# nubot-nudt/LCR-Net

Measured on AMD Instinct MI355X. Metric: scans/s (120k-pt KITTI-shape scan -> 256-D descriptor), higher is better.
Workload: dtype f32 (K-deep GEMMs, K >= 288 and N >= 64: fp32 operands as bf16 x 3 split, 6 of 9 products on the bf16 matrix cores, fp32 accumulate — error vs fp64 <= the fp32-MFMA kernel's; every other GEMM, KPConv and attention: fp32 MFMA); 1 GPU; configs[1]: batch of 8 synthetic 64-beam scans (~120k pts, 0.3 m voxel -> ~16k pts), voxelise + 3 subsamples + 10 radius searches + KPConv encoder + NetVLAD, seeded random weights; distinct_input_batches=4, streams=pre-processing stream (own host thread, 2 batches ahead) + 2 encoder stream(s), parallelism=scan-parallel x1, all-gather of descriptors

## Files before the change

### include/lcr_hip.h

```cpp
#ifndef LCR_HIP_H
#define LCR_HIP_H
#include <stddef.h>
#include <stdint.h>
#ifdef __cplusplus
extern "C" {
#endif

#define LCR_OK 0
#define LCR_EARG (-1)
#define LCR_ESPACE (-2)
#define LCR_EHIP (-3)

#define LCR_STATUS_KEY_OVERFLOW 1u
#define LCR_STATUS_LEN_MISMATCH 2u
#define LCR_GN_REPLICAS 8

const char* lcr_last_error(void);
void lcr_ktimer_enable(int on);
void lcr_ktimer_sample(int every);
void lcr_ktimer_kinds(unsigned mask);
int lcr_ktimer_read(int kind, int max_records, double* seconds, int64_t* meta);
int lcr_ktimer_read2(int kind, int max_records, double* seconds, double* seconds_kernel, int64_t* meta);
int lcr_stream_spin(int microseconds, void* stream);
int lcr_version(void);
// ... 86 lines not shown
int lcr_gemm_f32_bsplit_masked(const float* A, const uint16_t* Bs_tiles, float* C, int64_t M, int N, int K, const float* bias,
                               const float* rowdiv, const int64_t* seg_len, int S, int groups, double* stats, const uint16_t* row_mask,
                               int block_k, void* stream);
int lcr_kpconv_mask_ok(int64_t M, int N, int K, int split);
int lcr_gemm_f32_anorm(const float* A, const float* B, float* C, int64_t M, int N, int K, const float* bias,
                       const double* a_stats, const float* a_gamma, const float* a_beta, int a_groups, float a_eps,
                       float a_slope, const int64_t* seg_len, int S, int groups, double* stats, void* stream);
int lcr_gemm_f32_bsplit_anorm(const float* A, const uint16_t* Bs_tiles, float* C, int64_t M, int N, int K, const float* bias,
                              const double* a_stats, const float* a_gamma, const float* a_beta, int a_groups, float a_eps,
                              float a_slope, const int64_t* seg_len, int S, int groups, double* stats, void* stream);
int lcr_gemm_split_ok(int N, int K);
int lcr_gemm_f32_batched_ta(const float* A, const float* B, float* C, int64_t M, int N, int count, const int* k_host,
                            const int64_t* a_off_host, const int64_t* b_off_host, const int64_t* c_off_host, void* stream);
int lcr_kpconv_aggregate(const float* s_feats, const uint8_t* s_pos, const float* q_pts, const float* s_pts,
                         const void* idx, int idx_is_64, int64_t M, int64_t Ns, int H, int C,
                         const float* kernel_points_host, float sigma, float* A, float* nn,
                         const int32_t* order , void* stream);
#define LCR_KP_VALID_FIRST 1
int lcr_kpconv_aggregate_ex(const float* s_feats, const uint8_t* s_pos, const float* q_pts, const float* s_pts,
                            const void* idx, int idx_is_64, int64_t M, int64_t Ns, int H, int C,
                            const float* kernel_points_host, float sigma, float* A, float* nn,
                            const int32_t* order, int flags, void* stream);
int lcr_kpconv_aggregate_mask(const float* s_feats, const uint8_t* s_pos, const float* q_pts, const float* s_pts,
                              const void* idx, int idx_is_64, int64_t M, int64_t Ns, int H, int C,
                              const float* kernel_points_host, float sigma, float* A, float* nn, uint16_t* mask,
                              const int32_t* order, int flags, void* stream);
int lcr_kpconv_fused(const float* s_feats, const uint8_t* s_pos, const float* q_pts, const float* s_pts, const void* idx,
                     int idx_is_64, int64_t M, int64_t Ns, int H, int C, const float* kernel_points_host, float sigma,
                     const float* W, const float* bias, float* out, const int64_t* seg_len, int S, int groups, double* stats,
                     const int32_t* order, void* stream);
int lcr_kpconv_cin1(const float* s_feats, const float* q_pts, const float* s_pts, const void* idx, int idx_is_64,
                    int64_t M, int64_t Ns, int H, const float* kernel_points_host, float sigma, const float* W,
                    const float* bias, int Cout, float* out, const int32_t* order, void* stream);
int lcr_maxpool(const float* x, const void* idx, int idx_is_64, int64_t M, int64_t Ns, int H, int C, float* out,
                const int32_t* order, void* stream);
int lcr_row_positive(const float* x, int64_t N, int C, uint8_t* pos, void* stream);
int lcr_groupnorm_stats(const float* x, int64_t N, int C, int groups, const int64_t* seg_len, int S, double* stats, void* stream);
int lcr_groupnorm_apply(const float* x, const double* stats, const float* gamma, const float* beta, const float* res,
                        const double* res_stats, const float* res_gamma, const float* res_beta, float* y, int64_t N, int C,
                        int groups, const int64_t* seg_len, int S, float eps, float slope, int act, uint8_t* pos, void* stream);

#define LCR_ENC_BLOCKS 10
typedef struct LcrUnaryW {
  const float *w, *b;
  const float *gn_w, *gn_b;
  const uint16_t* w_split;
} LcrUnaryW;
typedef struct LcrBlockW {
  int   cin, cout, strided;
  float sigma;
  const float* kernel_points_host;
  const float *kp_w, *kp_b;
  const float* kp_wt;
  const uint16_t* kp_wt_split;
  const float *normconv_w, *normconv_b;
  LcrUnaryW unary1, unary2, shortcut;
} LcrBlockW;
typedef struct LcrEncoderW {
  int   groups, c1_cout;
  float c1_sigma;
  const float* c1_kernel_points_host;
  const float *c1_w, *c1_b;
  const float *c1_gn_w, *c1_gn_b;
  LcrBlockW blocks[LCR_ENC_BLOCKS];
} LcrEncoderW;
int lcr_encoder_ws_bytes(const LcrEncoderW* W, const int64_t* n_host, int S, size_t* bytes);
// ... 222 lines not shown
```

### include/lcr_hip_debug.h

```cpp
#ifndef LCR_HIP_DEBUG_H
#define LCR_HIP_DEBUG_H

#ifdef __cplusplus
extern "C" {
#endif

void lcr_gemm_debug_force_tile(int tile);
void lcr_gemm_debug_deep(int mode);
void lcr_gemm_debug_streamk(int mode);
void lcr_groupnorm_debug_general(int on);
void lcr_kpconv_debug_off64(int on);

#ifdef __cplusplus
}
#endif
#endif
```

### lcr-net_amd/_lib.py

```python
import ctypes
import os
import re
import types

import torch

_PKG = os.path.dirname(os.path.abspath(__file__))
LIB_PATH = os.path.join(_PKG, "liblcr_hip.so")

_lib = None

HEADERS = [os.path.join(_PKG, "..", "include", h) for h in ("lcr_hip.h", "lcr_hip_debug.h")]
_SCALARS = {"int": ctypes.c_int, "int64_t": ctypes.c_int64, "uint32_t": ctypes.c_uint32, "uint64_t": ctypes.c_uint64, "unsigned": ctypes.c_uint,
            "size_t": ctypes.c_size_t, "float": ctypes.c_float, "double": ctypes.c_double}
_RESULTS = {"int": ctypes.c_int, "void": None, "const char*": ctypes.c_char_p}


def parse_header(text):
    text = re.sub(r"/\*.*?\*/|//[^\n]*", " ", text, flags=re.S)
    text = re.sub(r"^\s*#.*$", "", text, flags=re.M)
    sigs = {}
    for m in re.finditer(r"\b(lcr_\w+)\s*\(", text):
        name = m.group(1)
        head = text[:m.start()]
        res = re.sub(r"\s*\*", "*", " ".join(head[max(head.rfind(c) for c in ";{}") + 1:].split()))
        tail = re.match(r"([^()]*)\)\s*;", text[m.end():])
        if res not in _RESULTS or tail is None:
            raise RuntimeError("%s: cannot parse its prototype (result type %r)" % (name, res))
        args = []
        for p in ([] if tail.group(1).strip() in ("", "void") else tail.group(1).split(",")):
            words = re.sub(r"\bconst\b", " ", p).split()
            ctype = ctypes.c_void_p if "*" in p else _SCALARS.get(" ".join(words[:-1] if len(words) > 1 else words))
            if ctype is None:
                raise RuntimeError("%s: parameter %r has no ctypes mapping" % (name, " ".join(p.split())))
            args.append(ctype)
        sigs[name] = (_RESULTS[res], args)
    return sigs


_RELEASES_GIL = {"lcr_roformer_forward", "lcr_precompute_batch", "lcr_precompute_batch_rows", "lcr_precompute_batch_rows_ex", "lcr_hashmap_bucket_host", "lcr_encoder_forward", "lcr_encoder_forward_ex", "lcr_ktimer_read",
                 "lcr_ktimer_read2", "lcr_hashmap_order_host", "lcr_ransac_sample_host", "lcr_icp_point_to_point", "lcr_icp_point_to_plane", "lcr_netvlad_forward", "lcr_log_sinkhorn", "lcr_log_sinkhorn_ex",
                 "lcr_local_global_registration", "lcr_local_global_registration_ex", "lcr_retrieval_topk", "lcr_stream_spin"}


def build():
    import importlib.util
    spec = importlib.util.spec_from_file_location("_lcr_build", os.path.join(_PKG, "csrc", "build.py"))
    mod = importlib.util.module_from_spec(spec)
    spec.loader.exec_module(mod)
    return mod.build()


_RETURNS_VALUE = {"lcr_version", "lcr_kpconv_mask_ok", "lcr_gemm_split_ok", "lcr_ktimer_read", "lcr_ktimer_read2"}


def __getattr__(name):
    if name == "call":
        lib()
        return call
    raise AttributeError(name)


def _raise_on_rc(rc, fn, args):
    if rc:
        check(rc, fn.__name__)
    return rc


def lib():
    global _lib, call
    if _lib is None:
        if not os.path.exists(LIB_PATH):
            raise RuntimeError(
                "liblcr_hip.so not found at %s — build it with `python lcr-net_amd/csrc/build.py` "
                "(there is no CPU fallback for the lcr-net_amd hot path)" % LIB_PATH)
        sigs = {}
        for header in HEADERS:
            with open(header) as f:
                sigs.update(parse_header(f.read()))
        L = ctypes.CDLL(LIB_PATH)
        K = ctypes.PyDLL(LIB_PATH) if os.environ.get("LCR_CTYPES_KEEP_GIL", "1") != "0" else L
        checked = types.SimpleNamespace()
        for name, (res, args) in sigs.items():
            if not hasattr(L, name):
                continue
            dll = L if name in _RELEASES_GIL else K
# ... 46 lines not shown
```

### lcr-net_amd/csrc/encoder.hip

```cpp
#include <algorithm>
#include <cstdlib>
#include <cstring>

#include "common.h"

#define TURN(call) ([&]() { LaunchTurn turn_; return (call); }())

namespace lcr {

constexpr float ENC_GN_EPS = 1e-5f;
constexpr float ENC_SLOPE = 0.1f;

struct Arena {
  char*  base;
  size_t off, cap;
  template <typename T>
  T* take(size_t n) {
    const size_t o = off;
    off = align_up(off + n * sizeof(T));
    return (base && off <= cap) ? reinterpret_cast<T*>(base + o) : nullptr;
  }
};

struct StageIO {
  const float*   pts;
  const int64_t* seg;
  const int32_t* order;
  int64_t        n;
  int64_t        min_rows;
};

struct StatsPool {
  double* base;
  size_t  off, cap;
  int     S, groups;
  double* take() {
    const size_t n = static_cast<size_t>(GN_REPLICAS) * S * groups * 2;
    if (off + n > cap) return nullptr;
    double* p = base + off;
    off += n;
    return p;
  }
};

static size_t stats_doubles(int S, int groups) { return static_cast<size_t>(GN_REPLICAS) * S * groups * 2 * 44; }

static int unary_raw(const LcrUnaryW& u, const float* x, int64_t n, int cin, int cout, const StageIO& st, StatsPool& sp, Arena& ws,
                     float** y_out, double** stats_out, hipStream_t s) {
  float* y = ws.take<float>(static_cast<size_t>(n) * cout);
  double* stats = sp.take();
  if (!y || !stats) return LCR_ESPACE;
  const bool split = u.w_split && lcr_gemm_split_ok(cout, cin);
  int rc = split ? TURN(lcr_gemm_f32_bsplit(x, u.w_split, y, n, cout, cin, u.b, nullptr, st.seg, sp.S, sp.groups, stats, s))
                 : TURN(lcr_gemm_f32(x, u.w, y, n, cout, cin, 0, 1, u.b, nullptr, st.seg, sp.S, sp.groups, stats, s));
  *y_out = y;
  *stats_out = stats;
  return rc;
}

static int residual_block(const LcrBlockW& b, const float* s_feats, const StageIO& q, const StageIO& sup, const void* idx, int H,
                          StatsPool& sp, Arena& ws, float* out, unsigned enc_flags, hipStream_t s) {
  const int mid = b.cout / 4, g = sp.groups;
  const int64_t M = q.n, Ns = sup.n;
  int rc;
  const float* x = s_feats;
  uint8_t* pos = ws.take<uint8_t>(static_cast<size_t>(Ns));
  if (!pos) return LCR_ESPACE;
  if (b.unary1.w) {
    float* y1;
    double* st1;
    if ((rc = unary_raw(b.unary1, s_feats, Ns, b.cin, mid, sup, sp, ws, &y1, &st1, s))) return rc;
    float* x1 = ws.take<float>(static_cast<size_t>(Ns) * mid);
    if (!x1) return LCR_ESPACE;
    if ((rc = TURN(lcr_groupnorm_apply(y1, st1, b.unary1.gn_w, b.unary1.gn_b, nullptr, nullptr, nullptr, nullptr, x1, Ns, mid, g, sup.seg, sp.S,
                                  ENC_GN_EPS, ENC_SLOPE, 1, pos, s))))
      return rc;
    x = x1;
  } else if ((rc = TURN(lcr_row_positive(s_feats, Ns, b.cin, pos, s)))) {
    return rc;
  }
  float* A = ws.take<float>(static_cast<size_t>(M) * 15 * mid);
  float* nn = ws.take<float>(static_cast<size_t>(M));
  float* kpo = ws.take<float>(static_cast<size_t>(M) * mid);
  uint16_t* kmask = ws.take<uint16_t>(static_cast<size_t>(M));
  double* stc = sp.take();
  if (!A || !nn || !kpo || !kmask || !stc) return LCR_ESPACE;
  static const bool vf_env_off = getenv("LCR_KP_VALID_FIRST") && atoi(getenv("LCR_KP_VALID_FIRST")) == 0;
  const int vf_flag = ((enc_flags & LCR_ENC_LISTS_VALID_FIRST) && !vf_env_off) ? LCR_KP_VALID_FIRST : 0;
  static const bool fused32 = getenv("LCR_KPCONV_FUSED") != nullptr;
  if (fused32 && mid == 32 && sp.S <= 64) {
    if ((rc = TURN(lcr_kpconv_fused(x, pos, q.pts, sup.pts, idx, 0, M, Ns, H, mid, b.kernel_points_host, b.sigma, b.kp_w, b.kp_b, kpo, q.seg, sp.S, g,
                                    stc, q.order, s))))
      return rc;
  } else {
    const bool split = b.kp_wt_split && mid >= 64;
    if (!((split || b.kp_wt) && lcr_kpconv_mask_ok(M, mid, 15 * mid, split))) kmask = nullptr;
    if ((rc = TURN(lcr_kpconv_aggregate_mask(x, pos, q.pts, sup.pts, idx, 0, M, Ns, H, mid, b.kernel_points_host, b.sigma, A, nn, kmask, q.order, vf_flag,
                                             s))))
      return rc;
    if (split) {
      if ((rc = TURN(kmask ? lcr_gemm_f32_bsplit_masked(A, b.kp_wt_split, kpo, M, mid, 15 * mid, b.kp_b, nn, q.seg, sp.S, g, stc, kmask, mid, s)
                           : lcr_gemm_f32_bsplit(A, b.kp_wt_split, kpo, M, mid, 15 * mid, b.kp_b, nn, q.seg, sp.S, g, stc, s))))
        return rc;
    } else if (kmask) {
      if ((rc = TURN(lcr_gemm_f32_masked(A, b.kp_wt, kpo, M, mid, 15 * mid, b.kp_b, nn, q.seg, sp.S, g, stc, kmask, mid, s)))) return rc;
    } else if ((rc = TURN(b.kp_wt ? lcr_gemm_f32(A, b.kp_wt, kpo, M, mid, 15 * mid, 0, 1, b.kp_b, nn, q.seg, sp.S, g, stc, s)
                                  : lcr_gemm_f32(A, b.kp_w, kpo, M, mid, 15 * mid, 0, 0, b.kp_b, nn, q.seg, sp.S, g, stc, s)))) return rc;
  }
  float* y;
  double* sty;
  static const bool no_anorm = getenv("LCR_NO_NORM_ON_LOAD") != nullptr;
  if (!no_anorm && mid <= 256 && mid % 4 == 0 && b.cout > 32 && q.min_rows >= 64) {
    y = ws.take<float>(static_cast<size_t>(M) * b.cout);
    sty = sp.take();
    if (!y || !sty) return LCR_ESPACE;
    const bool split2 = b.unary2.w_split && lcr_gemm_split_ok(b.cout, mid);
    if ((rc = split2 ? TURN(lcr_gemm_f32_bsplit_anorm(kpo, b.unary2.w_split, y, M, b.cout, mid, b.unary2.b, stc, b.normconv_w, b.normconv_b, g,
                                                      ENC_GN_EPS, ENC_SLOPE, q.seg, sp.S, g, sty, s))
                     : TURN(lcr_gemm_f32_anorm(kpo, b.unary2.w, y, M, b.cout, mid, b.unary2.b, stc, b.normconv_w, b.normconv_b, g, ENC_GN_EPS,
                                               ENC_SLOPE, q.seg, sp.S, g, sty, s))))
      return rc;
// ... 73 lines not shown
                                      const int64_t* n_host, const int64_t* seg_min_rows_host, const int* limits, float* const* out_feats,
                                      unsigned flags, void* ws, size_t ws_bytes, void* stream) {
  if (!W || !feats0 || !points || !neighbors || !subsampling || !seg_len || !n_host || !limits || !out_feats || !ws || S < 1) {
    set_error("lcr_encoder_forward: bad argument");
    return LCR_EARG;
  }
  size_t need = 0;
  lcr_encoder_ws_bytes(W, n_host, S, &need);
  if (ws_bytes < need) {
    set_error("lcr_encoder_forward: workspace too small (%zu < %zu)", ws_bytes, need);
    return LCR_ESPACE;
  }
  hipStream_t s = static_cast<hipStream_t>(stream);
  StageIO st[4];
  for (int i = 0; i < 4; ++i) st[i] = StageIO{points[i], seg_len[i], order ? order[i] : nullptr, n_host[i], seg_min_rows_host ? seg_min_rows_host[i] : 0};
  Arena top{static_cast<char*>(ws), 0, ws_bytes};
  StatsPool sp{top.take<double>(stats_doubles(S, W->groups)), 0, stats_doubles(S, W->groups), S, W->groups};
  size_t pp = 0;
  for (int i = 0; i < LCR_ENC_BLOCKS; ++i) pp = std::max(pp, sizeof(float) * static_cast<size_t>(n_host[BLOCK_Q[i]]) * W->blocks[i].cout);
  pp = std::max(pp, sizeof(float) * static_cast<size_t>(n_host[0]) * W->c1_cout * 2);
  float* ping = reinterpret_cast<float*>(top.take<char>(pp));
  float* pong = reinterpret_cast<float*>(top.take<char>(pp));
  const size_t scratch0 = top.off;
  if (!sp.base || !ping || !pong) return LCR_ESPACE;
  hipMemsetAsync(sp.base, 0, sizeof(double) * sp.cap, s);

  int rc;
  float* cur;
  {
    const int64_t n0 = n_host[0];
    float* raw = ping;
    float* f = ping + static_cast<size_t>(n0) * W->c1_cout;
    double* stt = sp.take();
    if ((rc = TURN(lcr_kpconv_cin1(feats0, st[0].pts, st[0].pts, neighbors[0], 0, n0, n0, limits[0], W->c1_kernel_points_host, W->c1_sigma, W->c1_w,
                              W->c1_b, W->c1_cout, raw, st[0].order, s))))
      return rc;
    if ((rc = TURN(lcr_groupnorm_stats(raw, n0, W->c1_cout, W->groups, st[0].seg, S, stt, s)))) return rc;
    if ((rc = TURN(lcr_groupnorm_apply(raw, stt, W->c1_gn_w, W->c1_gn_b, nullptr, nullptr, nullptr, nullptr, f, n0, W->c1_cout, W->groups, st[0].seg, S,
                                  ENC_GN_EPS, ENC_SLOPE, 1, nullptr, s))))
      return rc;
    cur = f;
  }
  static const int STAGE_LAST[4] = {0, 3, 6, 9};
  for (int i = 0; i < LCR_ENC_BLOCKS; ++i) {
    const int qs = BLOCK_Q[i], ss = BLOCK_S[i];
    const bool strided = qs != ss;
    const void* idx = strided ? static_cast<const void*>(subsampling[ss]) : static_cast<const void*>(neighbors[qs]);
    const int H = limits[ss];
    float* out = nullptr;
    for (int k = 0; k < 4; ++k)
      if (STAGE_LAST[k] == i) out = out_feats[k];
    if (!out) out = (cur >= ping && cur < ping + pp / sizeof(float)) ? pong : ping;
    Arena scratch{static_cast<char*>(ws), scratch0, ws_bytes};
    if ((rc = residual_block(W->blocks[i], cur, st[qs], st[ss], idx, H, sp, scratch, out, flags, s))) {
      if (rc == LCR_ESPACE) set_error("lcr_encoder_forward: block %d ran out of workspace", i);
      return rc;
    }
    cur = out;
  }
  return check_launch("lcr_encoder_forward");
}
```

### lcr-net_amd/csrc/kpconv.hip

```cpp
#include <algorithm>
#include <cstdlib>

#include "common.h"

namespace lcr {

constexpr int KP_K = 15;
constexpr int KP_HMAX = 128;
constexpr int KP_WAVES = 4;

struct KPoints {
  float p[KP_K][3];
};

__device__ __forceinline__ void wave_lds_sync() {
  __builtin_amdgcn_fence(__ATOMIC_RELEASE, "wavefront");
  __builtin_amdgcn_wave_barrier();
  __builtin_amdgcn_fence(__ATOMIC_ACQUIRE, "wavefront");
}

typedef float floatx4 __attribute__((ext_vector_type(4)));

struct XcdBand {
  int64_t begin, end, stride;
// ... 466 lines not shown
      for (int i = 0; i < 4; ++i) b4[i] = (u4 ? b8[i + 4] : b8[i]) + __shfl_xor(u4 ? b8[i] : b8[i + 4], 16);
#pragma unroll
      for (int i = 0; i < 2; ++i) b2[i] = (u3 ? b4[i + 2] : b4[i]) + __shfl_xor(u3 ? b4[i] : b4[i + 2], 8);
      b1 = (u2 ? b2[1] : b2[0]) + __shfl_xor(u2 ? b2[0] : b2[1], 4);
      b1 += __shfl_xor(b1, 2);
      b1 += __shfl_xor(b1, 1);
      if ((lane & 3) == 0) s_a[w][(u5 ? 8 : 0) + (u4 ? 4 : 0) + (u3 ? 2 : 0) + (u2 ? 1 : 0)] = b1;
    }
    wave_lds_sync();
    const float cntf = s_a[w][15];
    const float div = cntf > 1.f ? cntf : 1.f;
    float av[KP_K];
#pragma unroll
    for (int k = 0; k < KP_K; ++k) av[k] = s_a[w][k];
#pragma unroll
    for (int q = 0; q < MAXO; ++q) {
      const int o = lane + 64 * q;
      if (o < Cout) {
        float v = 0.f;
#pragma unroll
        for (int k = 0; k < KP_K; ++k) v = fmaf(av[k], wreg[q][k], v);
        v = v / div;
        if (bias) v += breg[q];
        out[m * Cout + o] = v;
      }
    }
    wave_lds_sync();
    r0 = r1;
    n0 = n1;
    r1 = r2;
  }
}

template <typename IdxT>
__global__ __launch_bounds__(256) void k_maxpool(const float* __restrict__ x, const IdxT* __restrict__ idx, int64_t M, int64_t Ns, int H, int C,
                                                 float* __restrict__ out, const int32_t* __restrict__ order) {
  __shared__ int32_t s_idx[4][KP_HMAX];
  const int lane = threadIdx.x & 63, w = __builtin_amdgcn_readfirstlane(threadIdx.x >> 6);
  const XcdBand band = xcd_band(M, w, 4);
  for (int64_t t = band.begin; t < band.end; t += band.stride) {
    const int64_t m = order ? order[t] : t;
    int n = 0;
    bool any_shadow = false;
    for (int h0 = 0; h0 < H; h0 += 64) {
      const int h = h0 + lane;
      int64_t j = Ns;
      if (h < H) j = static_cast<int64_t>(idx[m * H + h]);
      const bool ok = j >= 0 && j < Ns;
      const uint64_t mk = wave_ballot(ok);
      if (ok) s_idx[w][n + mbcnt_lt(mk)] = static_cast<int32_t>(j);
      any_shadow |= (wave_ballot(h < H && !ok) != 0ull);
      n += __popcll(mk);
    }
    wave_lds_sync();
    const float init = any_shadow ? 0.f : -INFINITY;
    if ((C & 255) == 0) {
      for (int c = lane * 4; c < C; c += 256) {
        float4 v = make_float4(init, init, init, init);
        for (int h0 = 0; h0 < n; h0 += 8) {
          float4 f[8];
#pragma unroll
          for (int u = 0; u < 8; ++u)
            f[u] = *reinterpret_cast<const float4*>(x + static_cast<int64_t>(s_idx[w][h0 + u < n ? h0 + u : n - 1]) * C + c);
#pragma unroll
          for (int u = 0; u < 8; ++u) {
            v.x = fmaxf(v.x, f[u].x);
// ... 130 lines not shown
                                const float* W, const float* bias, float* out, const int64_t* seg_len, int S, int groups, double* stats,
                                const int32_t* order, void* stream) {
  if (!s_feats || !s_pos || !q_pts || !s_pts || !idx || !kernel_points_host || !W || !out || M < 0 || Ns < 0 || H < 1 || H > KP_HMAX ||
      !(sigma > 0.f) || C != KF_C) {
    set_error("lcr_kpconv_fused: bad argument (C must be %d, H in [1,%d])", KF_C, KP_HMAX);
    return LCR_EARG;
  }
  if (stats && (!seg_len || S < 1 || S > KF_MAX_SEG || groups < 1 || C % groups != 0)) {
    set_error("lcr_kpconv_fused: statistics need seg_len, 1 <= S <= %d and groups dividing C", KF_MAX_SEG);
    return LCR_EARG;
  }
  if (M == 0) return LCR_OK;
  const KPoints kp = load_kp(kernel_points_host);
  hipStream_t st = static_cast<hipStream_t>(stream);
  KernelTimerScope timed(KT_KPCONV_FUSED, st, M, Ns, H, C, idx_is_64 ? 8 : 4);
  static const int n_cu = [] {
    int dev = 0, cus = 0;
    if (hipGetDevice(&dev) != hipSuccess || hipDeviceGetAttribute(&cus, hipDeviceAttributeMultiprocessorCount, dev) != hipSuccess || cus <= 0)
      cus = 256;
    return cus;
  }();
  const int64_t tiles_per_band = ((M + 7) / 8 + KF_Q - 1) / KF_Q;
  const int grid = 8 * static_cast<int>(std::max<int64_t>(1, std::min<int64_t>(tiles_per_band, (3 * n_cu + 7) / 8)));
  const int Sx = stats ? S : 1;
  if (idx_is_64)
    hipLaunchKernelGGL((k_kpconv_fused32<int64_t>), dim3(grid), dim3(KP_WAVES * 64), 0, st, s_feats, s_pos, q_pts, s_pts,
                       static_cast<const int64_t*>(idx), M, Ns, H, kp, sigma, W, bias, out, stats ? seg_len : nullptr, Sx, groups, stats, order);
  else
    hipLaunchKernelGGL((k_kpconv_fused32<int32_t>), dim3(grid), dim3(KP_WAVES * 64), 0, st, s_feats, s_pos, q_pts, s_pts,
                       static_cast<const int32_t*>(idx), M, Ns, H, kp, sigma, W, bias, out, stats ? seg_len : nullptr, Sx, groups, stats, order);
  return check_launch("lcr_kpconv_fused");
}

extern "C" int lcr_kpconv_cin1(const float* s_feats, const float* q_pts, const float* s_pts, const void* idx, int idx_is_64, int64_t M,
                               int64_t Ns, int H, const float* kernel_points_host, float sigma, const float* W, const float* bias, int Cout,
                               float* out, const int32_t* order, void* stream) {
  if (!s_feats || !q_pts || !s_pts || !idx || !kernel_points_host || !W || !out || M < 0 || H < 1 || Cout < 1 || Cout > 256 || !(sigma > 0.f)) {
    set_error("lcr_kpconv_cin1: bad argument");
    return LCR_EARG;
  }
  if (M == 0) return LCR_OK;
  const KPoints kp = load_kp(kernel_points_host);
  hipStream_t st = static_cast<hipStream_t>(stream);
  dim3 grid(grid_for_xcd(M, KP_WAVES)), block(KP_WAVES * 64);
#define LCR_CIN1(IDX, MAXO) \
  hipLaunchKernelGGL((k_kpconv_cin1<IDX, MAXO>), grid, block, 0, st, s_feats, q_pts, s_pts, static_cast<const IDX*>(idx), M, Ns, H, kp, sigma, W, bias, Cout, out, order)
  if (idx_is_64) {
    if (Cout <= 64) LCR_CIN1(int64_t, 1);
    else LCR_CIN1(int64_t, 4);
  } else {
    if (Cout <= 64) LCR_CIN1(int32_t, 1);
    else LCR_CIN1(int32_t, 4);
  }
#undef LCR_CIN1
  return check_launch("lcr_kpconv_cin1");
}

extern "C" int lcr_maxpool(const float* x, const void* idx, int idx_is_64, int64_t M, int64_t Ns, int H, int C, float* out,
                           const int32_t* order, void* stream) {
  if (!x || !idx || !out || M < 0 || H < 1 || H > KP_HMAX || C < 1) {
    set_error("lcr_maxpool: bad argument");
    return LCR_EARG;
  }
  if (M == 0) return LCR_OK;
  hipStream_t st = static_cast<hipStream_t>(stream);
  dim3 grid(grid_for_xcd(M, 4)), block(256);
  if (idx_is_64) hipLaunchKernelGGL((k_maxpool<int64_t>), grid, block, 0, st, x, static_cast<const int64_t*>(idx), M, Ns, H, C, out, order);
  else hipLaunchKernelGGL((k_maxpool<int32_t>), grid, block, 0, st, x, static_cast<const int32_t*>(idx), M, Ns, H, C, out, order);
  return check_launch("lcr_maxpool");
}

extern "C" int lcr_row_positive(const float* x, int64_t N, int C, uint8_t* pos, void* stream) {
  if (!x || !pos || N < 0 || C < 1) {
    set_error("lcr_row_positive: bad argument");
    return LCR_EARG;
  }
  if (N == 0) return LCR_OK;
  hipLaunchKernelGGL(k_row_pos, dim3(grid_for(N, 4)), dim3(256), 0, static_cast<hipStream_t>(stream), x, N, C, pos);
  return check_launch("lcr_row_positive");
}
```

### lcr-net_amd/functional.py

```python
import ctypes
import os
import threading

import numpy as np
import torch

from . import _lib

GN_EPS = 1e-5
GN_REPLICAS = 8


class KernelTimer:
    KINDS = {"gemm": 0, "kpconv_aggregate": 1, "radius_query": 2, "attention": 3, "kpconv_fused": 4, "sinkhorn": 5}

    def __init__(self, names):
        self.names = set(names)
        self._cache = None

    def summary(self):
        return {k: [(b, m) for b, _, m in v] for k, v in self.records().items()}

    def records(self):
        if self._cache is None:
# ... 306 lines not shown
            _lib.ptr(s_feats), _lib.ptr(s_pos), _lib.ptr(q_points), _lib.ptr(s_points), _lib.ptr(idx), _idx_args(idx), M, Ns, H, C,
            ctypes.c_void_p(kp.ctypes.data), float(sigma), _lib.ptr(A), _lib.ptr(nn), _lib.ptr(mask), _lib.ptr(order), 0,
            _lib.stream_ptr(s_feats.device))
        return A, nn, mask
    _lib.call.lcr_kpconv_aggregate(
        _lib.ptr(s_feats), _lib.ptr(s_pos), _lib.ptr(q_points), _lib.ptr(s_points), _lib.ptr(idx), _idx_args(idx), M, Ns, H, C,
        ctypes.c_void_p(kp.ctypes.data), float(sigma), _lib.ptr(A), _lib.ptr(nn), _lib.ptr(order), _lib.stream_ptr(s_feats.device))
    return A, nn


KPCONV_FUSED_C = 32


def kpconv_fused(s_feats, s_pos, q_points, s_points, idx, kernel_points_host, sigma, weights, bias, seg_len=None, groups=0, order=None):
    _lib.require_cuda(s_feats, q_points, s_points, idx)
    M, H = idx.shape
    Ns, C = s_feats.shape
    assert C == KPCONV_FUSED_C and tuple(weights.shape) == (15, C, C) and weights.is_contiguous()
    assert idx.is_contiguous() and s_feats.is_contiguous() and q_points.is_contiguous() and s_points.is_contiguous()
    out = torch.empty((M, C), dtype=torch.float32, device=s_feats.device)
    stats, S = None, 0
    if groups:
        seg_len = _seg(seg_len, M, s_feats.device)
        S = seg_len.numel()
        stats = _zero_stats(S, groups, s_feats.device)
    kp = _kp_host(kernel_points_host)
    _lib.call.lcr_kpconv_fused(
        _lib.ptr(s_feats), _lib.ptr(s_pos), _lib.ptr(q_points), _lib.ptr(s_points), _lib.ptr(idx), _idx_args(idx), M, Ns, H, C,
        ctypes.c_void_p(kp.ctypes.data), float(sigma), _lib.ptr(weights), _lib.ptr(bias), _lib.ptr(out),
        _lib.ptr(seg_len) if groups else None, S, int(groups), _lib.ptr(stats), _lib.ptr(order), _lib.stream_ptr(s_feats.device))
    return out, stats


def kpconv_cin1(s_feats, q_points, s_points, idx, kernel_points_host, sigma, weights, bias, order=None):
    M, H = idx.shape
    Ns = s_feats.shape[0]
    Cout = weights.shape[-1]
    out = torch.empty((M, Cout), dtype=torch.float32, device=s_feats.device)
    kp = _kp_host(kernel_points_host)
    _lib.call.lcr_kpconv_cin1(_lib.ptr(s_feats), _lib.ptr(q_points), _lib.ptr(s_points), _lib.ptr(idx), _idx_args(idx), M, Ns, H,
                              ctypes.c_void_p(kp.ctypes.data), float(sigma), _lib.ptr(weights), _lib.ptr(bias), Cout,
                              _lib.ptr(out), _lib.ptr(order), _lib.stream_ptr(s_feats.device))
    return out


def maxpool(x, idx, order=None):
    M, H = idx.shape
    out = torch.empty((M, x.shape[1]), dtype=torch.float32, device=x.device)
    _lib.call.lcr_maxpool(_lib.ptr(x), _lib.ptr(idx), _idx_args(idx), M, x.shape[0], H, x.shape[1], _lib.ptr(out),
                          _lib.ptr(order), _lib.stream_ptr(x.device))
    return out


class NetvladWeights(ctypes.Structure):
    _fields_ = [(n, ctypes.c_void_p) for n in (
        "cluster_weights", "cluster_weights2", "hidden1_weights", "bn1_w", "bn1_b", "bn1_mean", "bn1_var",
        "bn2_w", "bn2_b", "bn2_mean", "bn2_var", "gating_weights", "gbn_w", "gbn_b", "gbn_mean", "gbn_var")]


def netvlad_forward(feats, seg_len_host, weights_struct):
    _lib.require_cuda(feats)
    seg = np.ascontiguousarray(seg_len_host, dtype=np.int64)
    S = int(seg.shape[0])
    assert int(seg.sum()) == feats.shape[0] and feats.shape[1] == 1024 and feats.is_contiguous()
    ws = _lib.ws("lcr_netvlad_ws_bytes", feats.shape[0], S, device=feats.device)
    out = torch.empty((S, 256), dtype=torch.float32, device=feats.device)
    _lib.call.lcr_netvlad_forward(_lib.ptr(feats), ctypes.c_void_p(seg.ctypes.data), S, ctypes.byref(weights_struct),
                                  _lib.ptr(out), _lib.ptr(ws), ws.numel(), _lib.stream_ptr(feats.device))
    return out


def gemm_batched_ta(a, b, c, M, N, k, a_off, b_off, c_off):
    _lib.require_cuda(a, b, c)
    assert all(t.dtype == torch.float32 and t.is_contiguous() for t in (a, b, c))
    kk = np.ascontiguousarray(k, dtype=np.int32)
    ao, bo, co = (np.ascontiguousarray(v, dtype=np.int64) for v in (a_off, b_off, c_off))
# ... 970 lines not shown
```

### lcr-net_amd/modules/kpconv/kpconv.py

```python
import math
import os

import torch
import torch.nn as nn

from ... import functional as F
from ...weights import base_kernel_points


_FUSED = bool(os.environ.get("LCR_KPCONV_FUSED"))


class KPConv(nn.Module):
    def __init__(self, in_channels, out_channels, kernel_size, radius, sigma, bias=False, dimension=3, inf=1e6, eps=1e-9):
        super().__init__()
        assert kernel_size == 15 and dimension == 3, "the HIP path implements the 15-point rigid 3-D kernel of the reference config"
        self.kernel_size, self.in_channels, self.out_channels = kernel_size, in_channels, out_channels
        self.radius, self.sigma, self.dimension = radius, sigma, dimension
        self.inf, self.eps = inf, eps
        self.weights = nn.Parameter(torch.zeros(kernel_size, in_channels, out_channels))
        if bias:
            self.bias = nn.Parameter(torch.zeros(out_channels))
        else:
            self.register_parameter("bias", None)
# ... 11 lines not shown
        c = self._wt_cache
        if c is None or not c[0].same(w):
            with F.derived_lock:
                c = self._wt_cache
                if c is None or not c[0].same(w):
                    wt = w.detach().reshape(self.kernel_size * self.in_channels, self.out_channels).t().contiguous()
                    c = self._wt_cache = (F.WeightStamp(w), F.publish_derived(wt) if wt.is_cuda else wt)
        return c[1]

    def weights_t_split(self):
        wt = self.weights_t()
        c = getattr(self, "_wts_cache", None)
        if c is None or c[0] is not wt:
            with F.derived_lock:
                c = getattr(self, "_wts_cache", None)
                if c is None or c[0] is not wt:
                    c = self._wts_cache = (wt, F.publish_derived(F.split_bf16x3(wt)))
        return c[1]

    def kernel_points_host(self):
        kp = self.kernel_points
        c = self._kp_cache
        if c is None or not c[0].same(kp):
            c = self._kp_cache = (F.WeightStamp(kp), kp.detach().cpu().numpy().copy())
        return c[1]

    def _apply(self, fn, *args, **kwargs):
        F.drop_derived(self, "_kp_cache", "_wt_cache", "_wts_cache")
        return super()._apply(fn, *args, **kwargs)

    def forward_raw(self, s_feats, q_points, s_points, neighbor_indices, s_pos=None, seg_len=None, groups=0, order=None):
        kp = self.kernel_points_host()
        if self.in_channels == 1:
            out = F.kpconv_cin1(s_feats.contiguous().view(-1), q_points, s_points, neighbor_indices, kp, self.sigma,
                                self.weights, self.bias, order=order)
            stats = F.groupnorm_stats(out, groups, seg_len) if groups else None
            return out, stats
        if s_pos is None:
            s_pos = F.row_positive(s_feats)
        if (_FUSED and self.in_channels == self.out_channels == F.KPCONV_FUSED_C and neighbor_indices.shape[1] <= 128
                and (seg_len is None or seg_len.numel() <= 64)):
            return F.kpconv_fused(s_feats, s_pos, q_points, s_points, neighbor_indices, kp, self.sigma, self.weights, self.bias,
                                  seg_len=seg_len, groups=groups, order=order)
        wt = self.weights_t()
        split = F.gemm_split_enabled() and F.gemm_split_ok(wt.shape[0], wt.shape[1])
        M = neighbor_indices.shape[0]
        if F.kpconv_mask_ok(M, wt.shape[0], wt.shape[1], split):
            A, nn_cnt, mask = F.kpconv_aggregate(s_feats, s_pos, q_points, s_points, neighbor_indices, kp, self.sigma, order=order, emit_mask=True)
        else:
            (A, nn_cnt), mask = F.kpconv_aggregate(s_feats, s_pos, q_points, s_points, neighbor_indices, kp, self.sigma, order=order), None
        if split:
            return F.gemm_bsplit(A, self.weights_t_split(), bias=self.bias, rowdiv=nn_cnt, seg_len=seg_len, groups=groups, row_mask=mask)
        return F.gemm(A, wt, trans_b=True, bias=self.bias, rowdiv=nn_cnt, seg_len=seg_len, groups=groups, row_mask=mask)

    def forward(self, s_feats, q_points, s_points, neighbor_indices):
        return self.forward_raw(s_feats, q_points, s_points, neighbor_indices)[0]

    def __repr__(self):
        return (f"KPConv(kernel_size: {self.kernel_size}, in_channels: {self.in_channels}, out_channels: {self.out_channels}, "
                f"radius: {self.radius:g}, sigma: {self.sigma:g}, bias: {self.bias is not None})")
```

Baseline: 3105 scans/s.

## Add kernel-point-parallel first KPConv with valid-first early exit and optional fused GN stats

Adds a new first-layer (Cin=1) KPConv kernel that compacts valid neighbours into LDS per wave, spreads the 15 kernel points across lanes, and reduces with shuffles. It software-pipelines row loads and neighbour gathers and can stop scanning once a neighbour list runs out, when valid-first ordering is set. By default (form 1) it launches a grid capped per CU and still runs group-norm stats as a separate pass. Form 2 folds the stats into the kernel epilogue with split double atomics, trading extra atomics and a smaller grid for one fewer pass over the output.

```diff
diff --git a/include/lcr_hip.h b/include/lcr_hip.h
--- a/include/lcr_hip.h
+++ b/include/lcr_hip.h
@@ -142,6 +142,10 @@
 int lcr_kpconv_cin1(const float* s_feats, const float* q_pts, const float* s_pts, const void* idx, int idx_is_64,
                     int64_t M, int64_t Ns, int H, const float* kernel_points_host, float sigma, const float* W,
                     const float* bias, int Cout, float* out, const int32_t* order, void* stream);
+int lcr_kpconv_cin1_ex(const float* s_feats, const float* q_pts, const float* s_pts, const void* idx, int idx_is_64,
+                       int64_t M, int64_t Ns, int H, const float* kernel_points_host, float sigma, const float* W,
+                       const float* bias, int Cout, float* out, const int32_t* order, int flags, const int64_t* seg_len, int S,
+                       int groups, double* stats, void* stream);
 int lcr_maxpool(const float* x, const void* idx, int idx_is_64, int64_t M, int64_t Ns, int H, int C, float* out,
                 const int32_t* order, void* stream);
 int lcr_row_positive(const float* x, int64_t N, int C, uint8_t* pos, void* stream);
diff --git a/include/lcr_hip_debug.h b/include/lcr_hip_debug.h
--- a/include/lcr_hip_debug.h
+++ b/include/lcr_hip_debug.h
@@ -10,6 +10,9 @@
 void lcr_gemm_debug_streamk(int mode);
 void lcr_groupnorm_debug_general(int on);
 void lcr_kpconv_debug_off64(int on);
+void lcr_kpconv_debug_cin1_form(int form);
+void lcr_kpconv_debug_cin1_wg_per_cu(int n);
+int lcr_kpconv_debug_cin1_grid(int64_t M, int stats);
 
 #ifdef __cplusplus
 }
diff --git a/lcr-net_amd/_lib.py b/lcr-net_amd/_lib.py
--- a/lcr-net_amd/_lib.py
+++ b/lcr-net_amd/_lib.py
@@ -51,7 +51,7 @@
     return mod.build()
 
 
-_RETURNS_VALUE = {"lcr_version", "lcr_kpconv_mask_ok", "lcr_gemm_split_ok", "lcr_ktimer_read", "lcr_ktimer_read2"}
+_RETURNS_VALUE = {"lcr_version", "lcr_kpconv_mask_ok", "lcr_gemm_split_ok", "lcr_ktimer_read", "lcr_ktimer_read2", "lcr_kpconv_debug_cin1_grid"}
 
 
 def __getattr__(name):
diff --git a/lcr-net_amd/csrc/encoder.hip b/lcr-net_amd/csrc/encoder.hip
--- a/lcr-net_amd/csrc/encoder.hip
+++ b/lcr-net_amd/csrc/encoder.hip
@@ -56,6 +56,11 @@
   *y_out = y;
   *stats_out = stats;
   return rc;
+}
+
+static int kp_valid_first(unsigned enc_flags) {
+  static const bool vf_env_off = getenv("LCR_KP_VALID_FIRST") && atoi(getenv("LCR_KP_VALID_FIRST")) == 0;
+  return ((enc_flags & LCR_ENC_LISTS_VALID_FIRST) && !vf_env_off) ? LCR_KP_VALID_FIRST : 0;
 }
 
 static int residual_block(const LcrBlockW& b, const float* s_feats, const StageIO& q, const StageIO& sup, const void* idx, int H,
@@ -85,8 +90,7 @@
   uint16_t* kmask = ws.take<uint16_t>(static_cast<size_t>(M));
   double* stc = sp.take();
   if (!A || !nn || !kpo || !kmask || !stc) return LCR_ESPACE;
-  static const bool vf_env_off = getenv("LCR_KP_VALID_FIRST") && atoi(getenv("LCR_KP_VALID_FIRST")) == 0;
-  const int vf_flag = ((enc_flags & LCR_ENC_LISTS_VALID_FIRST) && !vf_env_off) ? LCR_KP_VALID_FIRST : 0;
+  const int vf_flag = kp_valid_first(enc_flags);
   static const bool fused32 = getenv("LCR_KPCONV_FUSED") != nullptr;
   if (fused32 && mid == 32 && sp.S <= 64) {
     if ((rc = TURN(lcr_kpconv_fused(x, pos, q.pts, sup.pts, idx, 0, M, Ns, H, mid, b.kernel_points_host, b.sigma, b.kp_w, b.kp_b, kpo, q.seg, sp.S, g,
@@ -226,10 +230,9 @@
     float* raw = ping;
     float* f = ping + static_cast<size_t>(n0) * W->c1_cout;
     double* stt = sp.take();
-    if ((rc = TURN(lcr_kpconv_cin1(feats0, st[0].pts, st[0].pts, neighbors[0], 0, n0, n0, limits[0], W->c1_kernel_points_host, W->c1_sigma, W->c1_w,
-                              W->c1_b, W->c1_cout, raw, st[0].order, s))))
-      return rc;
-    if ((rc = TURN(lcr_groupnorm_stats(raw, n0, W->c1_cout, W->groups, st[0].seg, S, stt, s)))) return rc;
+    if ((rc = TURN(lcr_kpconv_cin1_ex(feats0, st[0].pts, st[0].pts, neighbors[0], 0, n0, n0, limits[0], W->c1_kernel_points_host, W->c1_sigma, W->c1_w,
+                                 W->c1_b, W->c1_cout, raw, st[0].order, kp_valid_first(flags), st[0].seg, S, W->groups, stt, s))))
+      return rc;
     if ((rc = TURN(lcr_groupnorm_apply(raw, stt, W->c1_gn_w, W->c1_gn_b, nullptr, nullptr, nullptr, nullptr, f, n0, W->c1_cout, W->groups, st[0].seg, S,
                                   ENC_GN_EPS, ENC_SLOPE, 1, nullptr, s))))
       return rc;
diff --git a/lcr-net_amd/csrc/kpconv.hip b/lcr-net_amd/csrc/kpconv.hip
--- a/lcr-net_amd/csrc/kpconv.hip
+++ b/lcr-net_amd/csrc/kpconv.hip
@@ -522,6 +522,218 @@
   }
 }
 
+constexpr int KC_PAD = 4;
+
+template <bool STATS>
+__global__ __launch_bounds__(KP_WAVES * 64) void k_kpconv_cin1_kp(const float* __restrict__ s_feats, const float* __restrict__ q_pts,
+                                                                  const float* __restrict__ s_pts, const int32_t* __restrict__ idx, int64_t M,
+                                                                  int64_t Ns, int H, KPoints kp, float sigma, const float* __restrict__ W,
+                                                                  const float* __restrict__ bias, int Cout, float* __restrict__ out,
+                                                                  const int32_t* __restrict__ order, int valid_first,
+                                                                  const int64_t* __restrict__ seg_len, int S, int groups, double* __restrict__ stats) {
+  __shared__ __attribute__((aligned(16))) float4 s_rel[KP_WAVES][KP_HMAX + KC_PAD];
+  __shared__ __attribute__((aligned(16))) float s_a[KP_WAVES][16];
+  __shared__ int64_t s_start[STATS ? KF_MAX_SEG + 1 : 1];
+  __shared__ double s_fold[STATS ? KP_WAVES : 1][64][2];
+  __shared__ int s_fseg[KP_WAVES];
+  const int lane = threadIdx.x & 63, w = __builtin_amdgcn_readfirstlane(threadIdx.x >> 6);
+  const int sub = lane >> 4, col = lane & 15;
+  const float inv_sigma = 1.f / sigma;
+  float kx = 0.f, ky = 0.f, kz = 0.f;
+#pragma unroll
+  for (int k = 0; k < KP_K; ++k)
+    if (col == k) {
+      kx = kp.p[k][0];
+      ky = kp.p[k][1];
+      kz = kp.p[k][2];
+    }
+  float wreg[KP_K];
+#pragma unroll
+  for (int k = 0; k < KP_K; ++k) wreg[k] = lane < Cout ? W[k * Cout + lane] : 0.f;
+  const float breg = (bias && lane < Cout) ? bias[lane] : 0.f;
+  const uint32_t ns = static_cast<uint32_t>(Ns), hh = static_cast<uint32_t>(H);
+
+  double rs = 0.0, rss = 0.0;
+  int my_seg = -1;
+  int64_t seg_lo = 0, seg_hi = 0;
+  const int gs = STATS ? Cout / groups : 1;
+  static_assert(GN_REPLICAS == 8, "the replica pairs below are laid out for 8 replicas");
+  double* rep = STATS ? stats + static_cast<int64_t>(2 * (blockIdx.x & 3)) * S * groups * 2 : nullptr;
+  const int64_t rep_stride = static_cast<int64_t>(S) * groups * 2;
+  auto add_split = [&](double* d, double x) {
+    const double hi = __longlong_as_double(__double_as_longlong(x) & ~0x1fffffffll);
+    atomicAdd(d, hi);
+    atomicAdd(d + rep_stride, x - hi);
+  };
+  auto fold_group = [&](double& ds, double& dss) {
+    for (int d = 1; d < gs; d <<= 1) {
+      ds += __shfl_xor(ds, d);
+      dss += __shfl_xor(dss, d);
+    }
+  };
+  const bool group_lead = lane < Cout && (lane & (gs - 1)) == 0;
+  if constexpr (STATS) {
+    if (threadIdx.x == 0) {
+      int64_t o = 0;
+      for (int i = 0; i < S; ++i) {
+        s_start[i] = o;
+        o += seg_len[i];
+      }
+      s_start[S] = o;
+    }
+    __syncthreads();
+  }
+
+  const XcdBand band = xcd_band(M, w, KP_WAVES);
+  const int64_t stride = band.stride, M_end = band.end;
+  struct Row {
+    uint32_t m, ju;
+    float    qx, qy, qz;
+  };
+  struct Nb {
+    float f, x, y, z;
+  };
+  auto load_row = [&](int64_t tt, Row& r) {
+    const int64_t tc = tt < M_end ? tt : M_end - 1;
+    r.m = static_cast<uint32_t>(order ? order[tc] : static_cast<int32_t>(tc));
+    const float* q = reinterpret_cast<const float*>(reinterpret_cast<const char*>(q_pts) + r.m * 12u);
+    r.qx = q[0];
+    r.qy = q[1];
+    r.qz = q[2];
+    r.ju = lane < H ? static_cast<uint32_t>(idx[r.m * hh + static_cast<uint32_t>(lane)]) : ns;
+  };
+  auto gather = [&](const Row& r, Nb& nb) {
+    const uint32_t jc = r.ju < ns ? r.ju : 0u;
+    const float* sp = reinterpret_cast<const float*>(reinterpret_cast<const char*>(s_pts) + jc * 12u);
+    nb.f = s_feats[jc];
+    nb.x = sp[0];
+    nb.y = sp[1];
+    nb.z = sp[2];
+  };
+  int64_t t = band.begin;
+  if (t < M_end) {
+    Row r0, r1;
+    Nb n0, n1;
+    load_row(t, r0);
+    gather(r0, n0);
+    load_row(t + stride, r1);
+    for (; t < M_end; t += stride) {
+      Row r2;
+      gather(r1, n1);
+      load_row(t + 2 * stride, r2);
+      const uint32_t m = __builtin_amdgcn_readfirstlane(r0.m);
+      const float qx = r0.qx, qy = r0.qy, qz = r0.qz;
+      int n, cnt;
+      bool more;
+      {
+        const bool ok = r0.ju < ns;
+        const uint64_t mk = wave_ballot(ok);
+        if (ok) s_rel[w][mbcnt_lt(mk)] = make_float4(n0.x - qx, n0.y - qy, n0.z - qz, n0.f);
+        n = __popcll(mk);
+        cnt = __popcll(wave_ballot(ok && n0.f > 0.f));
+        more = !(valid_first && mk != ~0ull);
+      }
+      if (more) {
+        for (int h0 = 64; h0 < H; h0 += 64) {
+          const int h = h0 + lane;
+          const uint32_t ju = h < H ? static_cast<uint32_t>(idx[m * hh + static_cast<uint32_t>(h)]) : ns;
+          const bool ok = ju < ns;
+          const uint64_t mk = wave_ballot(ok);
+          float f = 0.f;
+          if (ok) {
+            const float* sp = reinterpret_cast<const float*>(reinterpret_cast<const char*>(s_pts) + ju * 12u);
+            f = s_feats[ju];
+            s_rel[w][n + mbcnt_lt(mk)] = make_float4(sp[0] - qx, sp[1] - qy, sp[2] - qz, f);
+          }
+          n += __popcll(mk);
+          cnt += __popcll(wave_ballot(ok && f > 0.f));
+          if (valid_first && mk != ~0ull) break;
+        }
+      }
+      if (lane < KC_PAD) s_rel[w][n + lane] = make_float4(1e6f, 1e6f, 1e6f, 0.f);
+      wave_lds_sync();
+      float a = 0.f;
+      {
+        const int steps = (n + 3) >> 2;
+        const float4* lp = &s_rel[w][sub];
+#pragma unroll 4
+        for (int s = 0; s < steps; ++s) {
+          const float4 p = lp[4 * s];
+          const float ex = p.x - kx, ey = p.y - ky, ez = p.z - kz;
+          const float wv = fmaxf(fmaf(-__builtin_amdgcn_sqrtf(fmaf(ez, ez, fmaf(ey, ey, ex * ex))), inv_sigma, 1.f), 0.f);
+          a = fmaf(wv, p.w, a);
+        }
+      }
+      a += __shfl_xor(a, 16);
+      a += __shfl_xor(a, 32);
+      if (lane < 16) s_a[w][lane] = a;
+      wave_lds_sync();
+      float av[16];
+#pragma unroll
+      for (int q = 0; q < 4; ++q) {
+        const float4 a4 = *reinterpret_cast<const float4*>(&s_a[w][4 * q]);
+        av[4 * q] = a4.x;
+        av[4 * q + 1] = a4.y;
+        av[4 * q + 2] = a4.z;
+        av[4 * q + 3] = a4.w;
+      }
+      float v = 0.f;
+#pragma unroll
+      for (int k = 0; k < KP_K; ++k) v = fmaf(av[k], wreg[k], v);
+      v = v / static_cast<float>(cnt > 1 ? cnt : 1);
+      if (bias) v += breg;
+      if (lane < Cout) out[static_cast<int64_t>(m) * Cout + lane] = v;
+      if constexpr (STATS) {
+        const int64_t m64 = m;
+        if (m64 < seg_lo || m64 >= seg_hi) {
+          if (my_seg >= 0) {
+            fold_group(rs, rss);
+            if (group_lead) {
+              double* d = rep + (static_cast<int64_t>(my_seg) * groups + lane / gs) * 2;
+              add_split(d, rs);
+              add_split(d + 1, rss);
+            }
+            rs = rss = 0.0;
+          }
+          int sg = 0;
+          while (sg + 1 < S && m64 >= s_start[sg + 1]) ++sg;
+          my_seg = sg;
+          seg_lo = s_start[sg];
+          seg_hi = s_start[sg + 1];
+        }
+        const double dv = lane < Cout ? static_cast<double>(v) : 0.0;
+        rs += dv;
+        rss += dv * dv;
+      }
+      wave_lds_sync();
+      r0 = r1;
+      n0 = n1;
+      r1 = r2;
+    }
+  }
+  if constexpr (STATS) {
+    fold_group(rs, rss);
+    s_fold[w][lane][0] = rs;
+    s_fold[w][lane][1] = rss;
+    if (lane == 0) s_fseg[w] = my_seg;
+    __syncthreads();
+    bool first = my_seg >= 0;
+    for (int ww = 0; ww < w; ++ww) first = first && s_fseg[ww] != my_seg;
+    if (first) {
+      for (int ww = w + 1; ww < KP_WAVES; ++ww)
+        if (s_fseg[ww] == my_seg) {
+          rs += s_fold[ww][lane][0];
+          rss += s_fold[ww][lane][1];
+        }
+      if (group_lead) {
+        double* d = rep + (static_cast<int64_t>(my_seg) * groups + lane / gs) * 2;
+        add_split(d, rs);
+        add_split(d + 1, rss);
+      }
+    }
+  }
+}
+
 template <typename IdxT>
 __global__ __launch_bounds__(256) void k_maxpool(const float* __restrict__ x, const IdxT* __restrict__ idx, int64_t M, int64_t Ns, int H, int C,
                                                  float* __restrict__ out, const int32_t* __restrict__ order) {
@@ -718,16 +930,72 @@
   return check_launch("lcr_kpconv_fused");
 }
 
+static int g_cin1_form = -1;
+extern "C" void lcr_kpconv_debug_cin1_form(int form) { g_cin1_form = form; }
+static int cin1_form() {
+  static const int env = [] {
+    const char* e = getenv("LCR_KPCONV_CIN1_FORM");
+    const int v = e ? atoi(e) : 1;
+    return (v == 0 || v == 2) ? v : 1;
+  }();
+  return g_cin1_form >= 0 ? g_cin1_form : env;
+}
+
+static int g_cin1_wg_per_cu = 0;
+extern "C" void lcr_kpconv_debug_cin1_wg_per_cu(int n) { g_cin1_wg_per_cu = n; }
+
+static int cin1_kp_grid(int64_t M, bool stats) {
+  static const int cus = [] {
+    int dev = 0, n = 0;
+    if (hipGetDevice(&dev) != hipSuccess || hipDeviceGetAttribute(&n, hipDeviceAttributeMultiprocessorCount, dev) != hipSuccess || n <= 0) n = 256;
+    return n;
+  }();
+  const int64_t cap = static_cast<int64_t>(cus) * (g_cin1_wg_per_cu > 0 ? g_cin1_wg_per_cu : stats ? 3 : 12);
+  const int64_t per_xcd = ((M + 7) / 8 + KP_WAVES - 1) / KP_WAVES;
+  return 8 * static_cast<int>(std::max<int64_t>(1, std::min<int64_t>(per_xcd, (cap + 7) / 8)));
+}
+extern "C" int lcr_kpconv_debug_cin1_grid(int64_t M, int stats) { return cin1_kp_grid(M, stats != 0); }
+
 extern "C" int lcr_kpconv_cin1(const float* s_feats, const float* q_pts, const float* s_pts, const void* idx, int idx_is_64, int64_t M,
                                int64_t Ns, int H, const float* kernel_points_host, float sigma, const float* W, const float* bias, int Cout,
                                float* out, const int32_t* order, void* stream) {
+  return lcr_kpconv_cin1_ex(s_feats, q_pts, s_pts, idx, idx_is_64, M, Ns, H, kernel_points_host, sigma, W, bias, Cout, out, order, 0, nullptr, 0, 0,
+                            nullptr, stream);
+}
+
+extern "C" int lcr_kpconv_cin1_ex(const float* s_feats, const float* q_pts, const float* s_pts, const void* idx, int idx_is_64, int64_t M,
+                                  int64_t Ns, int H, const float* kernel_points_host, float sigma, const float* W, const float* bias, int Cout,
+                                  float* out, const int32_t* order, int flags, const int64_t* seg_len, int S, int groups, double* stats,
+                                  void* stream) {
   if (!s_feats || !q_pts || !s_pts || !idx || !kernel_points_host || !W || !out || M < 0 || H < 1 || Cout < 1 || Cout > 256 || !(sigma > 0.f)) {
     set_error("lcr_kpconv_cin1: bad argument");
     return LCR_EARG;
   }
+  if (stats) {
+    const int gs = (groups >= 1 && Cout % groups == 0) ? Cout / groups : 0;
+    if (!seg_len || S < 1 || gs < 1 || (gs & (gs - 1)) != 0) {
+      set_error("lcr_kpconv_cin1: statistics need seg_len, S >= 1 and groups dividing Cout into power-of-two groups");
+      return LCR_EARG;
+    }
+  }
   if (M == 0) return LCR_OK;
   const KPoints kp = load_kp(kernel_points_host);
   hipStream_t st = static_cast<hipStream_t>(stream);
+  const int64_t lim = int64_t(1) << 30;
+  const int form = cin1_form();
+  if (form && !idx_is_64 && H <= KP_HMAX && Cout <= 64 && Ns > 0 && 3 * Ns < lim && 3 * M < lim && M * H < lim) {
+    const int vf = (flags & LCR_KP_VALID_FIRST) ? 1 : 0;
+    const bool in_epilogue = stats && form == 2 && S <= KF_MAX_SEG;
+    if (in_epilogue)
+      hipLaunchKernelGGL((k_kpconv_cin1_kp<true>), dim3(cin1_kp_grid(M, true)), dim3(KP_WAVES * 64), 0, st, s_feats, q_pts, s_pts,
+                         static_cast<const int32_t*>(idx), M, Ns, H, kp, sigma, W, bias, Cout, out, order, vf, seg_len, S, groups, stats);
+    else
+      hipLaunchKernelGGL((k_kpconv_cin1_kp<false>), dim3(cin1_kp_grid(M, false)), dim3(KP_WAVES * 64), 0, st, s_feats, q_pts, s_pts,
+                         static_cast<const int32_t*>(idx), M, Ns, H, kp, sigma, W, bias, Cout, out, order, vf, nullptr, 1, 1, nullptr);
+    const int rc = check_launch("lcr_kpconv_cin1");
+    if (rc != LCR_OK || !stats || in_epilogue) return rc;
+    return lcr_groupnorm_stats(out, M, Cout, groups, seg_len, S, stats, stream);
+  }
   dim3 grid(grid_for_xcd(M, KP_WAVES)), block(KP_WAVES * 64);
 #define LCR_CIN1(IDX, MAXO) \
   hipLaunchKernelGGL((k_kpconv_cin1<IDX, MAXO>), grid, block, 0, st, s_feats, q_pts, s_pts, static_cast<const IDX*>(idx), M, Ns, H, kp, sigma, W, bias, Cout, out, order)
@@ -739,7 +1007,9 @@
     else LCR_CIN1(int32_t, 4);
   }
 #undef LCR_CIN1
-  return check_launch("lcr_kpconv_cin1");
+  const int rc = check_launch("lcr_kpconv_cin1");
+  if (rc != LCR_OK || !stats) return rc;
+  return lcr_groupnorm_stats(out, M, Cout, groups, seg_len, S, stats, stream);
 }
 
 extern "C" int lcr_maxpool(const float* x, const void* idx, int idx_is_64, int64_t M, int64_t Ns, int H, int C, float* out,
diff --git a/lcr-net_amd/functional.py b/lcr-net_amd/functional.py
--- a/lcr-net_amd/functional.py
+++ b/lcr-net_amd/functional.py
@@ -362,16 +362,30 @@
     return out, stats
 
 
-def kpconv_cin1(s_feats, q_points, s_points, idx, kernel_points_host, sigma, weights, bias, order=None):
+KP_VALID_FIRST = 1
+
+
+def kpconv_cin1_ex(s_feats, q_points, s_points, idx, kernel_points_host, sigma, weights, bias, seg_len=None, groups=0, order=None,
+                   valid_first=False):
     M, H = idx.shape
     Ns = s_feats.shape[0]
     Cout = weights.shape[-1]
     out = torch.empty((M, Cout), dtype=torch.float32, device=s_feats.device)
+    stats, S = None, 0
+    if groups:
+        seg_len = _seg(seg_len, M, s_feats.device)
+        S = seg_len.numel()
+        stats = _zero_stats(S, groups, s_feats.device)
     kp = _kp_host(kernel_points_host)
-    _lib.call.lcr_kpconv_cin1(_lib.ptr(s_feats), _lib.ptr(q_points), _lib.ptr(s_points), _lib.ptr(idx), _idx_args(idx), M, Ns, H,
-                              ctypes.c_void_p(kp.ctypes.data), float(sigma), _lib.ptr(weights), _lib.ptr(bias), Cout,
-                              _lib.ptr(out), _lib.ptr(order), _lib.stream_ptr(s_feats.device))
-    return out
+    _lib.call.lcr_kpconv_cin1_ex(_lib.ptr(s_feats), _lib.ptr(q_points), _lib.ptr(s_points), _lib.ptr(idx), _idx_args(idx), M, Ns, H,
+                                 ctypes.c_void_p(kp.ctypes.data), float(sigma), _lib.ptr(weights), _lib.ptr(bias), Cout,
+                                 _lib.ptr(out), _lib.ptr(order), KP_VALID_FIRST if valid_first else 0,
+                                 _lib.ptr(seg_len) if groups else None, S, int(groups), _lib.ptr(stats), _lib.stream_ptr(s_feats.device))
+    return out, stats
+
+
+def kpconv_cin1(s_feats, q_points, s_points, idx, kernel_points_host, sigma, weights, bias, order=None):
+    return kpconv_cin1_ex(s_feats, q_points, s_points, idx, kernel_points_host, sigma, weights, bias, order=order)[0]
 
 
 def maxpool(x, idx, order=None):
diff --git a/lcr-net_amd/modules/kpconv/kpconv.py b/lcr-net_amd/modules/kpconv/kpconv.py
--- a/lcr-net_amd/modules/kpconv/kpconv.py
+++ b/lcr-net_amd/modules/kpconv/kpconv.py
@@ -67,10 +67,8 @@
     def forward_raw(self, s_feats, q_points, s_points, neighbor_indices, s_pos=None, seg_len=None, groups=0, order=None):
         kp = self.kernel_points_host()
         if self.in_channels == 1:
-            out = F.kpconv_cin1(s_feats.contiguous().view(-1), q_points, s_points, neighbor_indices, kp, self.sigma,
-                                self.weights, self.bias, order=order)
-            stats = F.groupnorm_stats(out, groups, seg_len) if groups else None
-            return out, stats
+            return F.kpconv_cin1_ex(s_feats.contiguous().view(-1), q_points, s_points, neighbor_indices, kp, self.sigma,
+                                    self.weights, self.bias, seg_len=seg_len, groups=groups, order=order)
         if s_pos is None:
             s_pos = F.row_positive(s_feats)
         if (_FUSED and self.in_channels == self.out_channels == F.KPCONV_FUSED_C and neighbor_indices.shape[1] <= 128
```

After: 3127 scans/s (median of 6 runs). Within noise of the previous version (+0.7%).
